# dfm/tinygp

Measured on AMD Instinct MI355X. Metric: GP log_probability evals/sec + Cholesky TFLOP/s (fp64), N=16,384, higher is better.
Workload: dtype f64; 1 GPU; c2: 1.5^2 ExpSquared(2.5), 1-D X, N=16384, fp64, diag=0.01, constant-density synthetic inputs (SURVEY 8d), dense Cholesky + tri-solve; n=16384, d=1, parallelism=single, nb_outer=1024

## Files before the change

tinygp_amd/csrc/capi.hip:

```cpp
#include <cmath>
#include <cstdlib>
#include <chrono>
#include <cstring>
#include <string>

#include "tgp_common.h"
#define CHAIN_HD __host__ __device__
#include "chain_tasks.h"
#define TILE_HD
#include "tile_order.h"

namespace tgp {

static thread_local std::string g_error;

void set_error(const char* fmt, ...) {
  char buf[1024];
  va_list ap;
  va_start(ap, fmt);
  vsnprintf(buf, sizeof(buf), fmt, ap);
  va_end(ap);
  g_error = buf;
}

// ... 239 lines not shown
  TGP_HIP_TRY(hipStreamSynchronize(ctx->stream));
  return TGP_OK;
}

static int64_t* option_slot(tgp_ctx* ctx, const char* key) {
  if (!strcmp(key, "nb_outer")) return &ctx->nb_outer;
  if (!strcmp(key, "lookahead")) return &ctx->lookahead;
  if (!strcmp(key, "profile")) return &ctx->profile;
  if (!strcmp(key, "first_split")) return &ctx->first_split;
  if (!strcmp(key, "first_small_tiles")) return &ctx->first_small_tiles;
  if (!strcmp(key, "keep_grad_buffers")) return &ctx->keep_grad_buffers;
  if (!strcmp(key, "stream_trsv")) return &ctx->stream_trsv;
  if (!strcmp(key, "trsv_groups")) return &ctx->trsv_groups;
  if (!strcmp(key, "nb_wide_rows")) return &ctx->nb_wide_rows;
  if (!strcmp(key, "dist_solve_aux")) return &ctx->dist_solve_aux;
  if (!strcmp(key, "solve_on_update")) return &ctx->solve_on_update;
  if (!strcmp(key, "fused_step")) return &ctx->fused_step;
  if (!strcmp(key, "chain_kernel")) return &ctx->chain_kernel;
  if (!strcmp(key, "chain_stamps")) return &ctx->chain_stamps;
  if (!strcmp(key, "chain_full_rows")) return &ctx->chain_full_rows;
  if (!strcmp(key, "chain_lds_pad")) return &ctx->chain_lds_pad;
  if (!strcmp(key, "chain_depth2")) return &ctx->chain_depth2;
  if (!strcmp(key, "chain_merged")) return &ctx->chain_merged;
  if (!strcmp(key, "chain_sub_panel")) return &ctx->chain_sub_panel;
  if (!strcmp(key, "chain_sub_min_rows")) return &ctx->chain_sub_min_rows;
  if (!strcmp(key, "chain_sub_role")) return &ctx->chain_sub_role;
  if (!strcmp(key, "chain_pre_wait")) return &ctx->chain_pre_wait;
  if (!strcmp(key, "chain_gate_split")) return &ctx->chain_gate_split;
  if (!strcmp(key, "chain_polls")) return &ctx->chain_polls;
  if (!strcmp(key, "chain_fwd_tasks")) return &ctx->chain_fwd_tasks;
  if (!strcmp(key, "chain_fast_update")) return &ctx->chain_fast_update;
  if (!strcmp(key, "chain_batch")) return &ctx->chain_batch;
  if (!strcmp(key, "chain_batch_lag")) return &ctx->chain_batch_lag;
  if (!strcmp(key, "chain_batch_rowlag")) return &ctx->chain_batch_rowlag;
  if (!strcmp(key, "chain_batch_minrows")) return &ctx->chain_batch_minrows;
  if (!strcmp(key, "kmat_plain_div")) return &ctx->kmat_plain_div;
  if (!strcmp(key, "chain_reserve")) return &ctx->chain_reserve;
  if (!strcmp(key, "gate_split")) return &ctx->gate_split;
  if (!strcmp(key, "reserve_max_tiles")) return &ctx->reserve_max_tiles;
  if (!strcmp(key, "sub_panel")) return &ctx->sub_panel;
  if (!strcmp(key, "sub_panel_min_rows")) return &ctx->sub_panel_min_rows;
  if (!strcmp(key, "nb_first")) return &ctx->nb_first;
  if (!strcmp(key, "split_tail")) return &ctx->split_tail;
  if (!strcmp(key, "gemm_role")) return &ctx->gemm_role;
  if (!strcmp(key, "host_join")) return &ctx->host_join;
  if (!strcmp(key, "late_join")) return &ctx->late_join;
// ... 998 lines not shown
```

tinygp_amd/csrc/chol.hip:

```cpp
#include <algorithm>
#include <atomic>
#include <functional>
#include <type_traits>

#include <thread>

#include "tgp_common.h"
#define CHAIN_HD __host__ __device__
#include "chain_tasks.h"

namespace tgp {

namespace {

typedef double d4 __attribute__((ext_vector_type(4)));
typedef float f4 __attribute__((ext_vector_type(4)));

template <typename T> struct Mfma;
template <> struct Mfma<double> {
  using acc_t = d4;
  static __device__ __forceinline__ acc_t mma(double a, double b, acc_t c) {
    return __builtin_amdgcn_mfma_f64_16x16x4f64(a, b, c, 0, 0, 0);
  }
  static __device__ __forceinline__ int drow(int lane, int r) { return (lane >> 4) + 4 * r; }
// ... 298 lines not shown
template <typename T> struct AgentBits;
template <> struct AgentBits<double> { using t = unsigned long long; };
template <> struct AgentBits<float> { using t = unsigned int; };
template <typename T>
__device__ __forceinline__ void st_agent(T* p, T v) {
  typename AgentBits<T>::t b;
  __builtin_memcpy(&b, &v, sizeof(T));
  __hip_atomic_store(reinterpret_cast<typename AgentBits<T>::t*>(p), b, __ATOMIC_RELAXED, __HIP_MEMORY_SCOPE_AGENT);
}

__device__ __forceinline__ void chain_stamp(long long* st, int k) {
  if (st != nullptr && threadIdx.x == 0) st[4 + k] = (long long)__builtin_amdgcn_s_memrealtime();
}

constexpr int CHAIN_FLAG_LD = 64;
constexpr uint32_t CHAIN_FINAL = 127;
constexpr int CHAIN_COLCNT_OFF = 16;
constexpr int CHAIN_QCNT_OFF = 96;
constexpr int CHAIN_XSTEP_OFF = 160;
constexpr int CHAIN_ZFLAG_OFF = 224;
constexpr int CHAIN_YSTATE_OFF = 288;
constexpr int CHAIN_TICKET_WORDS = CHAIN_YSTATE_OFF + int(CHAIN_MAX_ROW_TILES) / CHAIN_FWD_GROUP;
constexpr int CHAIN_PREFIX_OFF = CHAIN_TICKET_WORDS + 16;

template <typename T>
struct ChainArgs {
  T* A0;
  int64_t ld;
  T* dinv;
  int32_t* info;
  uint32_t* flags;
  int32_t* ticket;
  uint32_t epoch32;
  int32_t pivot_base;
  int32_t R;
  int32_t nblk;
  int32_t cb, ce;
  long long* stamps;
  int32_t launch;
  int32_t fast_update;
  const uint64_t* tasks;
  T* y;
  int32_t fgs;
  int32_t fprev;
  double* red;
  double* scal;
  int32_t red_total;
};

template <int NAP>
__device__ __forceinline__ void chain_wait(const uint32_t* f0, uint32_t v0, const uint32_t* f1, uint32_t v1,
                                           const uint32_t* f2, uint32_t v2, int32_t* info) {
  if (threadIdx.x < 64) {
    const int lane = threadIdx.x;
    const uint32_t* f = lane == 0 ? f0 : (lane == 1 ? f1 : (lane == 2 ? f2 : nullptr));
    const uint32_t want = lane == 0 ? v0 : (lane == 1 ? v1 : v2);
    bool ok = f == nullptr || __hip_atomic_load(f, __ATOMIC_RELAXED, __HIP_MEMORY_SCOPE_AGENT) == want;
    unsigned spin = 0;
    PollClock clk;
    while (!__all(ok)) {
      __builtin_amdgcn_s_sleep(NAP);
      if (!ok) ok = __hip_atomic_load(f, __ATOMIC_RELAXED, __HIP_MEMORY_SCOPE_AGENT) == want;
      bool dead = false;
      if ((spin & 255) == 255 && lane == 0)
        dead = clk.expired(spin) || poisoned(info);
      ++spin;
      if (__any(dead)) {
        if (lane == 0) atomicExch(info, STEP_TIMEOUT);
        break;
      }
    }
    if (lane == 0) __builtin_amdgcn_fence(__ATOMIC_ACQUIRE, "agent");
  }
  __syncthreads();
}

__device__ __forceinline__ void chain_publish(uint32_t* word, uint32_t value, int32_t* colcnt = nullptr) {
  asm volatile("s_waitcnt vmcnt(0)" ::: "memory");
  __syncthreads();
  if (threadIdx.x == 0) {
    __hip_atomic_store(word, value, __ATOMIC_RELAXED, __HIP_MEMORY_SCOPE_AGENT);
    if (colcnt != nullptr) __hip_atomic_fetch_add(colcnt, 1, __ATOMIC_RELAXED, __HIP_MEMORY_SCOPE_AGENT);
  }
}

// ... 782 lines not shown
    const ChainTask task = chain_unpack(q.tasks[t]);
    const int kind = task.kind, ti = task.i, tc = task.c, tk = task.k;
    s_task[5] = task.part;
    s_task[6] = task.k0;
    s_task[0] = kind; s_task[1] = ti; s_task[2] = tc; s_task[3] = tk;
  }
  __syncthreads();
  const int kind = __builtin_amdgcn_readfirstlane(s_task[0]);
  const int ti = __builtin_amdgcn_readfirstlane(s_task[1]);
  const int tc = __builtin_amdgcn_readfirstlane(s_task[2]);
  const int tk = __builtin_amdgcn_readfirstlane(s_task[3]);
  if (kind > 8) return;
  long long* st = nullptr;
  if (q.stamps != nullptr) {
    st = q.stamps + int64_t(__builtin_amdgcn_readfirstlane(s_task[4])) * 16;
    if (threadIdx.x == 0) {
      st[0] = kind; st[1] = kind == 1 ? tc : ti; st[2] = tc; st[3] = q.launch | (tk << 8) | (s_task[6] << 16);
      for (int k = 1; k < 12; ++k) st[4 + k] = 0;
    }
    chain_stamp(st, 0);
  }
  const uint32_t E = q.epoch32;
  const bool head_final = q.cb == 0;
  if (kind == 7) {
    const int c = tc;
    const int g = c / q.fgs;
    const bool prev = c > 0 || q.fprev != 0;
    chain_wait_counts(c - 1 > q.cb ? q.ticket + CHAIN_YSTATE_OFF + g : nullptr, c - 1 - q.cb,
                      (c == 0 && head_final) ? nullptr : reinterpret_cast<const int32_t*>(q.flags + c * CHAIN_FLAG_LD + c),
                      int32_t(E + CHAIN_FINAL), c > q.cb ? q.ticket + CHAIN_ZFLAG_OFF + (c - 1) : nullptr, 1, q.info);
    chain_stamp(st, 1);
    chain_fsolve<T>(q, S, c, prev);
    chain_stamp(st, 2);
    asm volatile("s_waitcnt vmcnt(0)" ::: "memory");
    __syncthreads();
    if (threadIdx.x == 0) __hip_atomic_store(q.ticket + CHAIN_ZFLAG_OFF + c, 1, __ATOMIC_RELAXED, __HIP_MEMORY_SCOPE_AGENT);
    chain_stamp(st, 3);
    return;
  }
  if (kind == 8) {
    const int c = tc, g = ti;
    const int target = q.R - c - ((c == 0 && head_final) ? 1 : 0);
    chain_wait_counts(q.ticket + CHAIN_COLCNT_OFF + c, target, q.ticket + CHAIN_ZFLAG_OFF + c, 1,
                      c > q.cb ? q.ticket + CHAIN_YSTATE_OFF + g : nullptr, c - q.cb, q.info);
    chain_stamp(st, 1);
    chain_fupdate<T>(q, S, c, g);
    chain_stamp(st, 2);
    asm volatile("s_waitcnt vmcnt(0)" ::: "memory");
    __syncthreads();
    if (threadIdx.x == 0)
      __hip_atomic_store(q.ticket + CHAIN_YSTATE_OFF + g, c - q.cb + 1, __ATOMIC_RELAXED, __HIP_MEMORY_SCOPE_AGENT);
    chain_stamp(st, 3);
    return;
  }
  if constexpr (sizeof(T) == 8) {
    if (kind == 6) {
      const int i = ti, c = tc, k = tk, k0 = __builtin_amdgcn_readfirstlane(s_task[6]);
      uint32_t* wt = q.flags + i * CHAIN_FLAG_LD + c;
      chain_wait<8>(q.flags + i * CHAIN_FLAG_LD + k, E + CHAIN_FINAL, q.flags + c * CHAIN_FLAG_LD + k, E + CHAIN_FINAL,
                    k0 > q.cb ? wt : nullptr, E + uint32_t(k0), q.info);
      chain_stamp(st, 1);
      chain_update_fast(q, S, i, c, k0, k + 1);
      chain_stamp(st, 2);
      chain_publish(wt, E + uint32_t(k + 1));
      chain_stamp(st, 3);
      return;
    }
  }
  if (kind >= 2 && kind <= 4) {
    const int i = ti, c = tc, k = tk;
    uint32_t* wt = q.flags + i * CHAIN_FLAG_LD + c;
    chain_wait<8>(q.flags + i * CHAIN_FLAG_LD + k, E + CHAIN_FINAL, q.flags + c * CHAIN_FLAG_LD + k, E + CHAIN_FINAL,
                  k > q.cb ? wt : nullptr, E + uint32_t(k), q.info);
    chain_stamp(st, 1);
    if (kind == 2) {
      if constexpr (sizeof(T) == 8) {
        if (q.fast_update) chain_update_fast(q, S, i, c, k, k + 1);
        else chain_update_full<T, 1>(q, S, i, c, k, 0);
      } else {
        chain_update_full<T, 1>(q, S, i, c, k, 0);
      }
    }
    else if (kind == 4) chain_update_full<T, CHAIN_CRIT_PARTS>(q, S, i, c, k, __builtin_amdgcn_readfirstlane(s_task[5]));
    else chain_update_diag<T>(q, S, c, k);
    chain_stamp(st, 2);
    if (kind == 4) {
      asm volatile("s_waitcnt vmcnt(0)" ::: "memory");
      __syncthreads();
      if (threadIdx.x == 0 &&
          __hip_atomic_fetch_add(q.ticket + CHAIN_QCNT_OFF + k, 1, __ATOMIC_RELAXED, __HIP_MEMORY_SCOPE_AGENT) ==
              CHAIN_CRIT_PARTS - 1)
        __hip_atomic_store(wt, E + uint32_t(k + 1), __ATOMIC_RELAXED, __HIP_MEMORY_SCOPE_AGENT);
    } else {
      chain_publish(wt, E + uint32_t(k + 1));
    }
    chain_stamp(st, 3);
    return;
  }
  __builtin_amdgcn_s_setprio(2);
  if (kind == 0) {
    const int i = ti, c = tc;
    uint32_t* wt = q.flags + i * CHAIN_FLAG_LD + c;
    const uint32_t* wl = q.flags + c * CHAIN_FLAG_LD + c;
    if (c > q.cb) chain_wait<4>(wt, E + uint32_t(c), nullptr, 0, nullptr, 0, q.info);
    acc_t V[8];
    chain_load_tile<T>(q, i, c, V);
    if (!(c == 0 && head_final)) chain_wait<4>(wl, E + CHAIN_FINAL, nullptr, 0, nullptr, 0, q.info);
    chain_stamp(st, 1);
    chain_solve<T>(q, S, i, c, V, st, 2);
    chain_publish(wt, E + CHAIN_FINAL, q.ticket + CHAIN_COLCNT_OFF + c);
    chain_stamp(st, 4);
    return;
  }
  const int c = tc;
  T* A = q.A0 + int64_t(c) * TILE * q.ld + int64_t(c) * TILE;
  const int64_t ld = q.ld;
  T* dinv = q.dinv + int64_t(c) * 2048;
  int32_t* info = q.info;
  const int32_t pivot_base = q.pivot_base + c * TILE;
  uint32_t* frow = q.flags + c * CHAIN_FLAG_LD;
  if (kind == 5) {
    acc_t Vx[8];
    if (c - 1 > q.cb) chain_wait<4>(frow + (c - 1), E + uint32_t(c - 1), nullptr, 0, nullptr, 0, q.info);
    chain_load_tile<T>(q, c, c - 1, Vx);
    chain_stamp(st, 1);
    const uint32_t* steps = c - 1 >= 1 ? q.flags + (c - 2) * CHAIN_FLAG_LD + (c - 1) : nullptr;
    int32_t* xstep = q.ticket + CHAIN_XSTEP_OFF + c;
    chain_xsolve_stream<T>(q, S, c, c - 1, Vx, steps, q.flags + (c - 1) * CHAIN_FLAG_LD + (c - 1), E, xstep);
    chain_stamp(st, 3);
    chain_publish(frow + (c - 1), E + CHAIN_FINAL, q.ticket + CHAIN_COLCNT_OFF + (c - 1));
    if (threadIdx.x == 0) __hip_atomic_store(xstep, 8, __ATOMIC_RELAXED, __HIP_MEMORY_SCOPE_AGENT);
    chain_stamp(st, 4);
    return;
  }
  acc_t Vx[8];
  acc_t Cfx[5];
  chain_fold_stream<T>(q, S, c, c - 1, Cfx, c > q.cb ? q.ticket + CHAIN_XSTEP_OFF + c : nullptr);
  chain_stamp(st, 3);
  if (c - 1 > q.cb) chain_wait<1>(frow + c, E + uint32_t(c - 1), nullptr, 0, nullptr, 0, q.info);
  else __syncthreads();
  chain_stamp(st, 5);
  {
    constexpr bool FOLD = true;
    uint32_t* step_word = q.flags + (c - 1) * CHAIN_FLAG_LD + c;
#define POTF2_ST(p, v) st_agent((p), T(v))
#define POTF2_V_IN_REGS Vx
#define POTF2_CF_IN_REGS Cfx
#define POTF2_PRE_SYNC(kb) do { if ((kb) >= 1) asm volatile("s_waitcnt vmcnt(0)" ::: "memory"); } while (0)
#define POTF2_POST_SYNC(kb)                                                                            \
  do {                                                                                                \
    if ((kb) >= 1 && threadIdx.x == 0)                                                                \
      __hip_atomic_store(step_word, E + uint32_t(kb), __ATOMIC_RELAXED, __HIP_MEMORY_SCOPE_AGENT);    \
  } while (0)
#include "potf2_body.inc"
#undef POTF2_POST_SYNC
#undef POTF2_PRE_SYNC
#undef POTF2_CF_IN_REGS
#undef POTF2_V_IN_REGS
#undef POTF2_ST
  }
  chain_stamp(st, 6);
  chain_publish(frow + c, E + CHAIN_FINAL, q.ticket + CHAIN_COLCNT_OFF + c);
// ... 721 lines not shown
  TGP_HIP_TRY(hipGetLastError());
  return TGP_OK;
}

template <typename T>
ChainPolicy chain_policy(const tgp_ctx* ctx) {
  if (sizeof(T) != 8 || ctx->chain_batch <= 1) return ChainPolicy{1, 1, 2, 0};
  return ChainPolicy{(int)ctx->chain_batch, (int)ctx->chain_batch_lag, (int)ctx->chain_batch_rowlag, (int)ctx->chain_batch_minrows};
}

template <typename T>
int launch_chain(tgp_ctx* ctx, hipStream_t st, T* A0, int64_t ld, T* dinv0, int64_t pivot_base, int64_t R,
                 int64_t nblk, int64_t cb, int64_t ce, bool head_done, hipEvent_t counters_ready, T* y0, bool fprev) {
  TGP_ARG_CHECK(R >= 1 && R <= CHAIN_MAX_ROW_TILES && cb >= 0 && cb < ce && ce <= nblk && nblk <= CHAIN_FLAG_LD && nblk <= R,
                "chain: bad panel shape (R=%lld, columns [%lld, %lld))", (long long)R, (long long)cb, (long long)ce);
  if (cb == 0 && !head_done) {
    TGP_TRY(launch_potf2<T>(ctx, st, A0, ld, dinv0, ctx->d_info, (int32_t)pivot_base));
    if (!ctx->trace) TGP_TRY(run_deferred_asm(ctx, st));
  }
  if (ctx->chain_polls_pending) {
    TGP_TRY(st_wait(ctx, st, ctx->ev_f));
    ctx->chain_polls_pending = false;
  }
  const int fwd = y0 != nullptr ? 1 : 0;
  int red = 0;
  if (fwd != 0 && ctx->chain_red_total > 0 && ctx->chain_red_total <= CHAIN_MAX_ROW_TILES && pivot_base % TILE == 0) {
    red = 1;
    ctx->chain_red_written += ce - cb;
    if (pivot_base / TILE + ce == ctx->chain_red_total && ctx->chain_red_written == ctx->chain_red_total) {
      red = 2;
      ctx->reductions_done = true;
    }
  }
  if (ctx->trace) {
    if (counters_ready != nullptr) TGP_TRY(ev_record(ctx, counters_ready, st));
    trace_push(ctx, 11, st, trace_off(ctx, A0), ld, R, cb, ce, nblk, fwd, red);
    return TGP_OK;
  }
  const ChainPolicy pol = chain_policy<T>(ctx);
  const std::array<int64_t, 9> key = {R, nblk, cb, ce, pol.batch, pol.lag, pol.rowlag, pol.minrows, fwd};
  auto found = ctx->chain_tables.find(key);
  if (found == ctx->chain_tables.end()) {
    const std::vector<ChainTask> list = chain_build((int)R, (int)nblk, (int)cb, (int)ce, pol, fwd, CHAIN_FWD_GROUP);
    tgp_ctx::ChainTable tab;
    tab.count = (int64_t)list.size();
    if (tab.count > 0) {
// ... 7 lines not shown
  const int64_t tasks = found->second.count;
  if (tasks == 0) {
    if (counters_ready != nullptr) TGP_TRY(ev_record(ctx, counters_ready, st));
    return TGP_OK;
  }
  ctx->step_epoch = (ctx->step_epoch + 1) & 0x1FFFFFFu;
  if (ctx->step_epoch == 0) ctx->step_epoch = 1;
  const uint32_t epoch = ctx->step_epoch;
  ChainArgs<T> q;
  q.A0 = A0; q.ld = ld; q.dinv = dinv0; q.info = ctx->d_info; q.flags = ctx->d_chain_flags;
  q.ticket = ctx->d_chain_ticket; q.epoch32 = epoch * 128u; q.pivot_base = (int32_t)pivot_base; q.R = (int32_t)R;
  q.nblk = (int32_t)nblk;
  q.cb = (int32_t)cb; q.ce = (int32_t)ce;
  q.stamps = nullptr;
  q.launch = (int32_t)ctx->chain_launches++;
  q.fast_update = (int32_t)ctx->chain_fast_update;
  q.tasks = found->second.dev;
  q.y = y0;
  q.fgs = CHAIN_FWD_GROUP;
  q.fprev = fprev ? 1 : 0;
  q.red = red != 0 ? ctx->d_chain_red : nullptr;
  q.scal = red != 0 ? ctx->d_scal : nullptr;
  q.red_total = red == 2 ? (int32_t)ctx->chain_red_total : 0;
  if (ctx->chain_stamps != 0 && ctx->chain_stamp_base + tasks <= CHAIN_STAMP_TASKS) {
    if (ctx->d_chain_stamps == nullptr)
      TGP_HIP_TRY(hipMalloc((void**)&ctx->d_chain_stamps, size_t(CHAIN_STAMP_TASKS) * 16 * sizeof(long long)));
    q.stamps = ctx->d_chain_stamps + ctx->chain_stamp_base * 16;
    ctx->chain_stamp_base += tasks;
  }
  TGP_HIP_TRY(hipMemsetAsync(ctx->d_chain_ticket, 0, size_t(CHAIN_TICKET_WORDS) * sizeof(int32_t), st));
  if (counters_ready != nullptr) TGP_TRY(ev_record(ctx, counters_ready, st));
  const size_t dyn = ctx->chain_lds_pad > 0 ? size_t(ctx->chain_lds_pad) + (sizeof(T) == 4 ? 36 * 256 * 4 : 0) : 0;
  hipLaunchKernelGGL((chain_kernel<T>), dim3((unsigned)tasks), dim3(512), dyn, st, q);
  TGP_HIP_TRY(hipGetLastError());
  return TGP_OK;
}

int launch_chain_poll(tgp_ctx* ctx, hipStream_t st, const void* A0, int64_t ld, int64_t R, int64_t c, bool first_external) {
  if (ctx->trace) {
    trace_push(ctx, 12, st, trace_off(ctx, static_cast<const double*>(A0)), ld, c);
    return TGP_OK;
  }
  const int32_t target = (int32_t)(R - c - ((c == 0 && first_external) ? 1 : 0));
  int32_t* count = ctx->d_chain_ticket + CHAIN_COLCNT_OFF + c;
  if (ctx->chain_polls == 3 && ctx->can_wait_value) {
    ctx->wait_values_inflight = true;
// ... 170 lines not shown
      if (S2 != S3 || !upd) TGP_TRY(st_wait(ctx, S2, ctx->ev_d));
      TGP_TRY(launch_trsv_fwd_step<T>(ctx, S2, mb, Ljj, ld, dj, y + j0));
    }
    if (need_mid) TGP_TRY(mid(ctx->ev_d));
    if (SB > 0 && j0 + TILE == sub_end && sub_end < k0 + kb) {
      const int64_t s0 = sub_end - SB, mr = n - sub_end, ncr = k0 + kb - sub_end;
      const T* P = A + s0 * ld + sub_end;
      const int64_t tiles = (mr / TILE) * (ncr / TILE) - (ncr / TILE) * (ncr / TILE - 1) / 2;
      TGP_TRY(launch_gemm_nt<T>(ctx, st, mr, ncr, SB, P, ld, P, ld, A + sub_end * ld + sub_end, ld, 1, 0,
                                tiles <= ctx->first_small_tiles ? 4 : 1));
    }
  }
  return TGP_OK;
}

template <typename T>
int potrf(tgp_ctx* ctx, int64_t n, T* A, int64_t ld, T* dinv, int32_t* info_host, T* y) {
  TGP_ARG_CHECK(n % TILE == 0 && ld >= n, "potrf: n must be a multiple of %d and ld >= n", TILE);
  if (info_host) *info_host = 0;
  if (n == 0) return TGP_OK;
  ctx->potf2_wait_counter = nullptr;
  ctx->prefix_hint_cols = 0;
  ctx->prefix_hint_counter = nullptr;
  ctx->reserve_hint = 0;
  hipStream_t S0 = ctx->stream, S1 = ctx->panel_stream;
  if (ctx->solve_on_update == 0 && y != nullptr) TGP_TRY(ensure_solve_stream(ctx));
  hipStream_t S2 = ctx->solve_on_update != 0 ? ctx->update_stream : ctx->solve_stream;
  if (y != nullptr) {
    TGP_TRY(ev_record(ctx, ctx->ev_c, S0));
    TGP_TRY(st_wait(ctx, S2, ctx->ev_c));
  }
  int64_t NB = ctx->nb_outer;
  if (NB < TILE) NB = TILE;
  NB = NB / TILE * TILE;
  if (!ctx->trace) TGP_HIP_TRY(hipMemsetAsync(ctx->d_info, 0, sizeof(int32_t), S0));
  ctx->chain_stamp_base = 0;
  ctx->chain_launches = 0;
  ctx->chain_polls_pending = false;
  const bool prof_on = ctx->profile != 0 && !ctx->trace;
  std::vector<ProfSpan> spans;
  ctx->ev_used = 0;
  hipEvent_t prof_t0 = nullptr;
  const bool span_dump = prof_on && getenv("TGP_SPAN_DUMP") != nullptr;
  if (prof_on) {
    TGP_TRY(prof_event(ctx, &prof_t0));
    TGP_HIP_TRY(hipEventRecord(prof_t0, S0));
// ... 65 lines not shown
    for (int64_t k0 = 0; k0 < n; k0 += width(k0)) s0.push_back(k0);
    s0.push_back(n);
    const int64_t P = (int64_t)s0.size() - 1;
    hipEvent_t ev_chain[2] = {ctx->ev_b, ctx->ev_g1}, ev_pfx[2] = {ctx->ev_g2, ctx->ev_e}, ev_T[2] = {ctx->ev_i, ctx->ev_j};
    const bool asm_side = ctx->asm_pending;
    ctx->asm_pending = false;
    if (P == 1 && !asm_side) {
      TGP_TRY(panel(S0, 0, s0[1] - s0[0], false, 0, no_mid));
      TGP_TRY(run_deferred_asm(ctx, nullptr));
    } else {
    TGP_TRY(ev_record(ctx, ctx->ev_a, S0));
    TGP_TRY(st_wait(ctx, S1, ctx->ev_a));
    TGP_TRY(panel(S1, 0, s0[1] - s0[0], false, 0, no_mid));
    TGP_TRY(run_deferred_asm(ctx, nullptr));
    TGP_TRY(ev_record(ctx, ev_chain[0], S1));
    for (int64_t p = 0; p + 1 < P; ++p) {
      const int64_t kb = s0[p + 1] - s0[p], next = s0[p + 1], wn = s0[p + 2] - s0[p + 1], mt = n - next;
      const T* Pp = A + s0[p] * ld + next;
      T* C = A + next * ld + next;
      TGP_TRY(st_wait(ctx, S0, ev_chain[p & 1]));
      if (p == 0 && asm_side) TGP_TRY(st_wait(ctx, S0, ctx->ev_asm));
      const bool prefix = wn < mt && ctx->chain_polls != 0;
      int32_t* counter = ctx->d_chain_ticket + CHAIN_PREFIX_OFF + (p & 3);
      if (prefix) {
        if (!ctx->trace) TGP_HIP_TRY(hipMemsetAsync(counter, 0, sizeof(int32_t), S0));
        TGP_TRY(ev_record(ctx, ev_pfx[p & 1], S0));
        ctx->prefix_hint_cols = wn;
        ctx->prefix_hint_counter = counter;
      }
      const int64_t t = mt / TILE;
      if (t * (t + 1) / 2 <= ctx->reserve_max_tiles) ctx->reserve_hint = ctx->chain_reserve;
      TGP_TRY(trailing(S0, mt, mt, kb, Pp, C, 0));
      if (!prefix) TGP_TRY(ev_record(ctx, ev_T[p & 1], S0));
      if (prefix) {
        const int64_t tm = mt / TILE, tp = wn / TILE;
        TGP_TRY(st_wait(ctx, S1, ev_pfx[p & 1]));
        if (ctx->trace || ctx->chain_polls == 2) {
          TGP_TRY(launch_prefix_poll(ctx, S1, counter, tp * tm - tp * (tp - 1) / 2, trace_off(ctx, C), ld));
        } else {
          ctx->potf2_wait_counter = counter;
          ctx->potf2_wait_target = tp * tm - tp * (tp - 1) / 2;
        }
      } else {
        TGP_TRY(st_wait(ctx, S1, ev_T[p & 1]));
      }
      if (p == 0 && asm_side) TGP_TRY(st_wait(ctx, S1, ctx->ev_asm));
      TGP_TRY(potf2_at(S1, next, false));
      TGP_TRY(chain_of_panel(S1, next, wn));
      TGP_TRY(ev_record(ctx, ev_chain[(p + 1) & 1], S1));
    }
    TGP_TRY(st_wait(ctx, S0, ev_chain[(P - 1) & 1]));
    }
  } else
  if (la && ctx->chain_kernel != 0 && ctx->chain_depth2 != 0) {
    std::vector<int64_t> s0;
    for (int64_t k0 = 0; k0 < n; k0 += width(k0)) s0.push_back(k0);
    s0.push_back(n);
    const int64_t P = (int64_t)s0.size() - 1;
    hipEvent_t ev_chain[2] = {ctx->ev_b, ctx->ev_g1}, ev_pre[2] = {ctx->ev_g2, ctx->ev_e};
    auto first_role = [&](int64_t m, int64_t nn) -> int {
      const int64_t tiles = (m / TILE) * (nn / TILE) - (nn / TILE) * (nn / TILE - 1) / 2;
      return tiles <= ctx->first_small_tiles ? 4 : 0;
    };
    const bool asm_side = ctx->asm_pending;
    ctx->asm_pending = false;
// ... 453 lines not shown
```

tinygp_amd/csrc/gemm.hip:

```cpp
#include <type_traits>

#include "tgp_common.h"

#define TILE_HD __host__ __device__
#include "tile_order.h"

namespace tgp {

namespace {

typedef double d4 __attribute__((ext_vector_type(4)));
typedef float f4 __attribute__((ext_vector_type(4)));

template <typename T> struct Mfma;
template <> struct Mfma<double> {
  using acc_t = d4;
  using v2_t = double __attribute__((ext_vector_type(2)));
  static __device__ __forceinline__ acc_t mma(double a, double b, acc_t c) {
    return __builtin_amdgcn_mfma_f64_16x16x4f64(a, b, c, 0, 0, 0);
  }
  static __device__ __forceinline__ int drow(int lane, int r) { return (lane >> 4) + 4 * r; }
};
template <> struct Mfma<float> {
  using acc_t = f4;
// ... 7 lines not shown
constexpr int BM = 128, BN = 128, BK = 16, LDS_LD = 144;

template <typename T>
struct GemmArgs {
  const T* A;
  const T* B;
  T* C;
  int64_t lda, ldb, ldc;
  int tm, tn;
  int k;
  int lower;
  int mode;
  int nblk;
  int skip00;
  int dG, dr, dl0, dnbt;
  int split_first, split_s, ngrid;
  T* ws;
  int* cnt;
  int batch;
  int64_t sA, sB, sC;
  int band;
  int prefix_tn = 0, prefix_cnt = 0;
  int32_t* prefix_done = nullptr;
};

__device__ __forceinline__ void decode_tile(int b, int tm, int tn, int lower, int& ti, int& tj, int band = 0) {
  tile_decode(b, tm, tn, lower, band, ti, tj);
}

template <typename T>
__device__ __forceinline__ void decode_tile_dist(int b, const GemmArgs<T>& g, int& ti, int& tj, int& gt) {
  int q = 0, g0 = (g.dl0 * g.dG + g.dr) * g.dnbt;
  const int step = g.dG * g.dnbt, tri = g.dnbt * (g.dnbt - 1) / 2;
  for (;;) {
    const int cnt = g.dnbt * (g.tm - g0) - tri;
    if (b < cnt) break;
    b -= cnt;
    g0 += step;
    ++q;
  }
  int tir, s;
  decode_tile(b, g.tm - g0, g.dnbt, 1, tir, s, g.band);
  ti = g0 + tir;
  tj = q * g.dnbt + s;
  gt = g0 + s;
}

template <typename T, int ROLE>
__global__ __launch_bounds__(256, 2) void gemm_nt_kernel(GemmArgs<T> g) {
  constexpr int SBUF = sizeof(T) == 8 ? 2 * BK * LDS_LD : 3 * BK * BM;
  __shared__ __attribute__((aligned(16))) T sAm[SBUF];
  __shared__ __attribute__((aligned(16))) T sBm[SBUF];
  T(*sA)[BK * LDS_LD] = reinterpret_cast<T(*)[BK * LDS_LD]>(sAm);
  T(*sB)[BK * LDS_LD] = reinterpret_cast<T(*)[BK * LDS_LD]>(sBm);

  if (ROLE == 1) __builtin_amdgcn_s_setprio(1);
  for (int tile = blockIdx.x; tile < (ROLE == 2 ? g.ngrid : g.nblk); tile += gridDim.x) {
  int bid = tile;
  int slice = 0, nsl = 1, tail_idx = 0;
  if (ROLE == 2 && tile >= g.split_first) {
    tail_idx = (tile - g.split_first) / g.split_s;
    slice = (tile - g.split_first) % g.split_s;
    nsl = g.split_s;
    bid = g.split_first + tail_idx;
  }
  const bool in_prefix = g.prefix_cnt > 0 && bid < g.prefix_cnt;
  {
    const int base = g.prefix_cnt > 0 ? (in_prefix ? 0 : g.prefix_cnt) : 0;
    const int cnt = g.prefix_cnt > 0 ? (in_prefix ? g.prefix_cnt : g.nblk - g.prefix_cnt) : g.nblk;
    const int loc = bid - base;
    const int nx = 8, q = cnt / nx, r = cnt % nx;
    const int xcd = loc % nx, idx = loc / nx;
    bid = base + (xcd < r ? xcd * (q + 1) : r * (q + 1) + (xcd - r) * q) + idx;
  }
  int ti, tj, gt;
  const T* gA = g.A;
  const T* gB = g.B;
  T* gC = g.C;
  if constexpr (ROLE == 3) {
    const int xcd = tile & 7, idx = tile >> 3, slot = idx & 63;
    const int pk = (idx >> 6) * 8 + xcd;
    const int ptm = (g.tm + 7) >> 3, ptn = (g.tn + 7) >> 3;
    const int pps = g.lower ? (ptm * (ptm + 1)) / 2 : ptm * ptn;
    const int pl = pk / g.batch, q = pk - pl * g.batch;
    if (pl >= pps) return;
    int Pi, Pj;
    if (g.lower) {
      Pi = int((sqrtf(8.0f * float(pl) + 1.0f) - 1.0f) * 0.5f);
      while (Pi > 0 && (Pi * (Pi + 1)) / 2 > pl) --Pi;
      while (((Pi + 1) * (Pi + 2)) / 2 <= pl) ++Pi;
// ... 181 lines not shown
#pragma unroll
          for (int b = 0; b < 4; ++b) {
            char* cb = const_cast<char*>(Cu) + (int64_t(a * 16) * g.ldc + b * 16) * 8;
#pragma unroll
            for (int t = 0; t < 4; ++t) *reinterpret_cast<double*>(cb + voff[t]) = cc[b][t];
          }
        }
      }
    } else
    if (pipe) {
      if (ROLE == 0 && in_prefix) {
#pragma unroll
        for (int a = 0; a < 4; ++a) {
#pragma unroll
          for (int b = 0; b < 4; ++b) {
            const char* cb = Cu + (int64_t(a * 16) * g.ldc + b * 16) * 8;
#pragma unroll
            for (int t = 0; t < 4; ++t)
              asm volatile("global_store_dwordx2 %0, %1, %2 sc1" ::"v"(voff[t]), "v"(acc[a][b][t]), "s"(cb) : "memory");
          }
        }
        asm volatile("s_waitcnt vmcnt(0)" ::: "memory");
        __syncthreads();
        if (tid == 0) __hip_atomic_fetch_add(g.prefix_done, 1, __ATOMIC_RELAXED, __HIP_MEMORY_SCOPE_AGENT);
      } else {
#pragma unroll
      for (int a = 0; a < 4; ++a) {
#pragma unroll
        for (int b = 0; b < 4; ++b) {
          char* cb = const_cast<char*>(Cu) + (int64_t(a * 16) * g.ldc + b * 16) * 8;
#pragma unroll
          for (int t = 0; t < 4; ++t) *reinterpret_cast<double*>(cb + voff[t]) = acc[a][b][t];
        }
      }
      }
    } else if (g.mode == 0) {
#pragma unroll
      for (int ap = 0; ap < 4; ap += 2) {
        T* col[2];
        double c[2][4][4];
#pragma unroll
        for (int a = 0; a < 2; ++a) {
          col[a] = Cb + int64_t((ap + a) * 16 + 4 * lq + lk) * g.ldc;
#pragma unroll
          for (int b = 0; b < 4; ++b)
#pragma unroll
            for (int t = 0; t < 4; ++t) c[a][b][t] = col[a][b * 16 + rot[t]];
// ... 98 lines not shown
              acc[a][b] = __builtin_amdgcn_mfma_f32_32x32x2f32(aop[a], bop[b], acc[a][b], 0, 0, 0);
        }
        stage = stage == NST - 1 ? 0 : stage + 1;
      }
    };
    kloop();
    if (g.mode == 0) {
#pragma unroll
      for (int a = 0; a < 2; ++a)
#pragma unroll
        for (int b = 0; b < 2; ++b) acc[a][b] = -acc[a][b];
    }
    if (ROLE == 0 && in_prefix) {
#pragma unroll
      for (int a = 0; a < 2; ++a)
#pragma unroll
        for (int b = 0; b < 2; ++b)
#pragma unroll
          for (int r = 0; r < 16; ++r)
            __hip_atomic_store(reinterpret_cast<uint32_t*>(centry(a, b, r)), __float_as_uint(acc[a][b][r]), __ATOMIC_RELAXED,
                               __HIP_MEMORY_SCOPE_AGENT);
      asm volatile("s_waitcnt vmcnt(0)" ::: "memory");
      __syncthreads();
      if (tid == 0) __hip_atomic_fetch_add(g.prefix_done, 1, __ATOMIC_RELAXED, __HIP_MEMORY_SCOPE_AGENT);
    } else {
#pragma unroll
    for (int a = 0; a < 2; ++a)
#pragma unroll
      for (int b = 0; b < 2; ++b)
#pragma unroll
        for (int r = 0; r < 16; ++r) *centry(a, b, r) = acc[a][b][r];
    }
  }
  }
}

constexpr int SM = 64, S_LD = 80;

template <typename T>
__global__ __launch_bounds__(256) __attribute__((amdgpu_waves_per_eu(3))) void gemm_nt_small_kernel(GemmArgs<T> g) {
  using M = Mfma<T>;
  using acc_t = typename M::acc_t;
  using v2_t = typename M::v2_t;
  constexpr int SBUF = sizeof(T) == 8 ? 3 * BK * SM : 2 * BK * S_LD;
  __shared__ __attribute__((aligned(16))) T sAm[SBUF];
  __shared__ __attribute__((aligned(16))) T sBm[SBUF];
  T(*sA)[BK * S_LD] = reinterpret_cast<T(*)[BK * S_LD]>(sAm);
// ... 246 lines not shown

}

static unsigned persistent_grid(const tgp_ctx* ctx, int nblk, int64_t reserve) {
  if (reserve <= 0) return unsigned(nblk);
  int64_t slots = 2 * int64_t(ctx->cus > 0 ? ctx->cus : 256) - reserve;
  slots = slots / 8 * 8;
  if (slots < 8) slots = 8;
  return unsigned(nblk <= slots ? nblk : slots);
}

template <typename T>
int launch_gemm_nt(tgp_ctx* ctx, hipStream_t st, int64_t m, int64_t n, int64_t k, const T* A,
                   int64_t lda, const T* B, int64_t ldb, T* C, int64_t ldc, int lower, int mode,
                   int role) {
  TGP_ARG_CHECK(m % BM == 0 && n % BN == 0 && k % BK == 0 && k > 0,
                "gemm_nt: m,n must be multiples of %d and k of %d (got %lld,%lld,%lld)", BM, BK,
                (long long)m, (long long)n, (long long)k);
  if (m == 0 || n == 0) return TGP_OK;
  if (ctx->trace) {
    const int64_t pfx = role == 0 ? ctx->prefix_hint_cols / BN : 0;
    ctx->prefix_hint_cols = 0;
    ctx->prefix_hint_counter = nullptr;
    if (role == 0) ctx->reserve_hint = 0;
    trace_push(ctx, 3, st, trace_off(ctx, A), trace_off(ctx, B), trace_off(ctx, C), m, n, k,
               int64_t(lower) | (int64_t(role) << 8) | (pfx << 16), ldc);
    return TGP_OK;
  }
  GemmArgs<T> g;
  g.skip00 = 0;
  g.dG = g.dr = g.dl0 = g.dnbt = 0;
  g.split_first = 0; g.split_s = 1; g.ngrid = 0; g.ws = nullptr; g.cnt = nullptr;
  g.batch = 1; g.sA = g.sB = g.sC = 0;
  g.band = (int)ctx->tile_band;
  g.prefix_tn = g.prefix_cnt = 0;
  g.prefix_done = nullptr;
  TGP_ARG_CHECK(role != 3 || (k <= 256 && mode == 0), "role 3 needs the small-tile path");
  if ((((role == 1 || role == 3) && k <= 256) || role == 4 || role == 5) && (mode == 0 || mode == 1)) {
    g.skip00 = (role == 3 || role == 5);
    g.A = A; g.B = B; g.C = C;
    g.lda = lda; g.ldb = ldb; g.ldc = ldc;
    g.tm = int(m / SM); g.tn = int(n / SM);
    g.k = int(k); g.lower = lower; g.mode = mode;
    if (lower) {
      if (g.tn > g.tm) g.tn = g.tm;
      g.nblk = g.tn * g.tm - (g.tn * (g.tn - 1)) / 2;
    } else {
      g.nblk = g.tm * g.tn;
    }
    hipLaunchKernelGGL((gemm_nt_small_kernel<T>), dim3((unsigned)g.nblk), dim3(256), 0, st, g);
    TGP_HIP_TRY(hipGetLastError());
    return TGP_OK;
  }
  g.A = A; g.B = B; g.C = C;
  g.lda = lda; g.ldb = ldb; g.ldc = ldc;
  g.tm = int(m / BM); g.tn = int(n / BN);
  g.k = int(k); g.lower = lower; g.mode = mode;
  if (lower) {
    if (g.tn > g.tm) g.tn = g.tm;
    g.nblk = g.tn * g.tm - (g.tn * (g.tn - 1)) / 2;
  } else {
    g.nblk = g.tm * g.tn;
  }
  const int64_t reserve = role == 0 ? ctx->reserve_hint : 0;
  ctx->reserve_hint = 0;
  if (role == 0 && ctx->prefix_hint_cols > 0) {
    TGP_ARG_CHECK(lower && mode == 0 && m == n && ctx->prefix_hint_cols % BN == 0 && ctx->prefix_hint_cols < n &&
                      k / BK >= 8 && ctx->prefix_hint_counter != nullptr,
                  "gemm_nt: a prefix needs a lower square update with at least 128 k-columns");
    g.prefix_tn = int(ctx->prefix_hint_cols / BN);
    g.prefix_cnt = tile_count(g.tm, g.prefix_tn, 1);
    g.prefix_done = ctx->prefix_hint_counter;
  }
  ctx->prefix_hint_cols = 0;
  ctx->prefix_hint_counter = nullptr;
  g.split_first = g.nblk; g.split_s = 1; g.ngrid = g.nblk; g.ws = nullptr; g.cnt = nullptr;
  if (ctx->split_tail != 0 && role == 0 && mode == 0 && reserve <= 0 && sizeof(T) == 8 && st == ctx->stream && g.prefix_cnt == 0) {
    const int slots = 2 * (ctx->cus > 0 ? ctx->cus : 256);
    const int R = g.nblk % slots, nkt = g.k / BK;
    int S = 1;
    while (R > 0 && 2 * S * R <= slots && 2 * S <= 8 && nkt % (2 * S) == 0 && nkt / (2 * S) >= 8) S *= 2;
    if (S > 1) {
      const size_t need = size_t(slots) * BM * BN * sizeof(T) + size_t(slots) * sizeof(int);
      if (ctx->gemm_ws_bytes < need) {
        if (ctx->d_gemm_ws) TGP_HIP_TRY(hipFree(ctx->d_gemm_ws));
        ctx->d_gemm_ws = nullptr;
        ctx->gemm_ws_bytes = 0;
        TGP_HIP_TRY(hipMalloc(&ctx->d_gemm_ws, need));
        TGP_HIP_TRY(hipMemset(ctx->d_gemm_ws, 0, need));
        ctx->gemm_ws_bytes = need;
      }
      g.split_first = g.nblk - R;
      g.split_s = S;
      g.ngrid = g.split_first + R * S;
      g.ws = static_cast<T*>(ctx->d_gemm_ws);
      g.cnt = reinterpret_cast<int*>(static_cast<char*>(ctx->d_gemm_ws) + size_t(slots) * BM * BN * sizeof(T));
      hipLaunchKernelGGL((gemm_nt_kernel<T, 2>), dim3(unsigned(g.ngrid)), dim3(256), 0, st, g);
      TGP_HIP_TRY(hipGetLastError());
// ... 128 lines not shown
```

tinygp_amd/csrc/tgp_common.h:

```cpp
#pragma once

#include <hip/hip_runtime.h>

#include <cstdarg>
#include <cstdint>
#include <cstdio>
#include <chrono>
#include <array>
#include <functional>
#include <map>
#include <mutex>
#include <vector>

#include "../../include/tgp_hip.h"

namespace tgp {

constexpr int TILE = TGP_TILE;
constexpr int SUB = 16;

void set_error(const char* fmt, ...);

#define TGP_HIP_TRY(expr)                                                                  \
  do {                                                                                     \
// ... 69 lines not shown
  int64_t trsv_groups = 0;
  int64_t keep_grad_buffers = 0;
  int64_t first_small_tiles = 1100;
  int64_t fused_step = 0;
  int64_t chain_reserve = 96;
  int64_t reserve_max_tiles = 1200;
  int64_t gate_split = 1;
  int64_t sub_panel = 0;
  int64_t sub_panel_min_rows = 0;
  int64_t nb_first = 0;
  int64_t split_tail = 0;
  int64_t gemm_role = 1;
  int64_t late_join = 1;
  int64_t chain_reduce = 1;
  double* d_chain_red = nullptr;
  int64_t chain_red_total = 0;
  int64_t chain_red_written = 0;
  bool reductions_done = false;
  bool defer_join = false;
  bool join_deferred = false;
  int64_t reserve_hint = 0;
  int64_t prefix_hint_cols = 0;
  int32_t* prefix_hint_counter = nullptr;
  const int32_t* potf2_wait_counter = nullptr;
  int64_t potf2_wait_target = 0;
  uint32_t* d_step_flag = nullptr;
  uint32_t step_epoch = 0;
  int64_t chain_kernel = 1;
  uint32_t* d_chain_flags = nullptr;
  int32_t* d_chain_ticket = nullptr;
  int64_t chain_fast_update = 0;
  int64_t chain_batch = 1;
  int64_t chain_batch_lag = 1;
  int64_t chain_batch_rowlag = 4;
  int64_t chain_batch_minrows = 32;
  struct ChainTable {
    uint64_t* dev = nullptr;
    int64_t count = 0;
  };
  std::map<std::array<int64_t, 9>, ChainTable> chain_tables;
  int64_t chain_full_rows = 4096;
  int64_t chain_depth2 = 1;
  int64_t chain_merged = 1;
  int64_t chain_sub_panel = 0;
  int64_t chain_sub_min_rows = 0;
  int64_t chain_sub_role = 4;
  int64_t kmat_plain_div = 0;
  int64_t chain_polls = 1;
  int64_t chain_fwd_tasks = 1;
  bool chain_fwd_now = false;
  bool wait_values_inflight = false;
  int64_t tile_band = 8;
  int64_t asm_defer = 0;
  std::function<int()> deferred_asm;
  hipEvent_t ev_asm_gate = nullptr;
  int64_t fault_inject = 0;
  int64_t host_join = 1;
  bool serializing_tool = false;
  hipStream_t rescue_stream = nullptr;
  hipEvent_t ev_join = nullptr;
  bool has_device = false;
  bool can_wait_value = false;
  int64_t poll_timeout_ms = 4000;
  int64_t timeout_retries = 0;
  int64_t chain_pre_wait = 0;
  int64_t chain_gate_split = 0;
// ... 227 lines not shown
```

Baseline: 39.85 evals/s.

## Gate tail chain tasks per column on trailing-update completion counters

For the last trailing update before the chained tail factorisation, the GEMM now bumps a per-column completion counter instead of a single prefix counter. The chain kernel starts without waiting for the whole update event, and each task polls its column's counter until all tiles in that column are done. This lets the tail Cholesky overlap with the end of the trailing GEMM rather than serialising on it. In exchange it adds extra polling lanes and atomics, and it disables the banded tile order for that launch.

New measurement: 39.96 evals/s (median of 6 runs). No clear change (+0.3%).

```diff
diff --git a/tinygp_amd/csrc/capi.hip b/tinygp_amd/csrc/capi.hip
--- a/tinygp_amd/csrc/capi.hip
+++ b/tinygp_amd/csrc/capi.hip
@@ -285,6 +285,8 @@
   if (!strcmp(key, "chain_lds_pad")) return &ctx->chain_lds_pad;
   if (!strcmp(key, "chain_depth2")) return &ctx->chain_depth2;
   if (!strcmp(key, "chain_merged")) return &ctx->chain_merged;
+  if (!strcmp(key, "chain_tail_prefix")) return &ctx->chain_tail_prefix;
+  if (!strcmp(key, "tail_prefix_launches")) return &ctx->tail_prefix_launches;
   if (!strcmp(key, "chain_sub_panel")) return &ctx->chain_sub_panel;
   if (!strcmp(key, "chain_sub_min_rows")) return &ctx->chain_sub_min_rows;
   if (!strcmp(key, "chain_sub_role")) return &ctx->chain_sub_role;
diff --git a/tinygp_amd/csrc/chol.hip b/tinygp_amd/csrc/chol.hip
--- a/tinygp_amd/csrc/chol.hip
+++ b/tinygp_amd/csrc/chol.hip
@@ -344,6 +344,8 @@
 constexpr int CHAIN_YSTATE_OFF = 288;
 constexpr int CHAIN_TICKET_WORDS = CHAIN_YSTATE_OFF + int(CHAIN_MAX_ROW_TILES) / CHAIN_FWD_GROUP;
 constexpr int CHAIN_PREFIX_OFF = CHAIN_TICKET_WORDS + 16;
+constexpr int CHAIN_COLGATE_OFF = CHAIN_PREFIX_OFF + 16;
+static_assert((CHAIN_COLGATE_OFF + CHAIN_FLAG_LD) * sizeof(int32_t) <= 4096, "d_chain_ticket is 4 096 bytes (capi.hip)");
 
 template <typename T>
 struct ChainArgs {
@@ -368,21 +370,27 @@
   double* red;
   double* scal;
   int32_t red_total;
+  const int32_t* gate;
 };
 
 template <int NAP>
 __device__ __forceinline__ void chain_wait(const uint32_t* f0, uint32_t v0, const uint32_t* f1, uint32_t v1,
-                                           const uint32_t* f2, uint32_t v2, int32_t* info) {
+                                           const uint32_t* f2, uint32_t v2, int32_t* info, const int32_t* fg = nullptr,
+                                           int32_t vg = 0) {
   if (threadIdx.x < 64) {
     const int lane = threadIdx.x;
-    const uint32_t* f = lane == 0 ? f0 : (lane == 1 ? f1 : (lane == 2 ? f2 : nullptr));
-    const uint32_t want = lane == 0 ? v0 : (lane == 1 ? v1 : v2);
-    bool ok = f == nullptr || __hip_atomic_load(f, __ATOMIC_RELAXED, __HIP_MEMORY_SCOPE_AGENT) == want;
+    const uint32_t* f = lane == 0 ? f0 : (lane == 1 ? f1 : (lane == 2 ? f2 : (lane == 3 ? reinterpret_cast<const uint32_t*>(fg) : nullptr)));
+    const uint32_t want = lane == 0 ? v0 : (lane == 1 ? v1 : (lane == 2 ? v2 : uint32_t(vg)));
+    auto ready = [&]() {
+      const uint32_t v = __hip_atomic_load(f, __ATOMIC_RELAXED, __HIP_MEMORY_SCOPE_AGENT);
+      return lane == 3 ? int32_t(v) >= int32_t(want) : v == want;
+    };
+    bool ok = f == nullptr || ready();
     unsigned spin = 0;
     PollClock clk;
     while (!__all(ok)) {
       __builtin_amdgcn_s_sleep(NAP);
-      if (!ok) ok = __hip_atomic_load(f, __ATOMIC_RELAXED, __HIP_MEMORY_SCOPE_AGENT) == want;
+      if (!ok) ok = ready();
       bool dead = false;
       if ((spin & 255) == 255 && lane == 0)
         dead = clk.expired(spin) || poisoned(info);
@@ -1211,6 +1219,9 @@
   }
   const uint32_t E = q.epoch32;
   const bool head_final = q.cb == 0;
+  const int gcol = kind == 5 ? tc - 1 : tc;
+  const int32_t* gate = (q.gate != nullptr && kind <= 6) ? q.gate + gcol : nullptr;
+  const int32_t gate_want = q.R - gcol;
   if (kind == 7) {
     const int c = tc;
     const int g = c / q.fgs;
@@ -1247,7 +1258,7 @@
       const int i = ti, c = tc, k = tk, k0 = __builtin_amdgcn_readfirstlane(s_task[6]);
       uint32_t* wt = q.flags + i * CHAIN_FLAG_LD + c;
       chain_wait<8>(q.flags + i * CHAIN_FLAG_LD + k, E + CHAIN_FINAL, q.flags + c * CHAIN_FLAG_LD + k, E + CHAIN_FINAL,
-                    k0 > q.cb ? wt : nullptr, E + uint32_t(k0), q.info);
+                    k0 > q.cb ? wt : nullptr, E + uint32_t(k0), q.info, gate, gate_want);
       chain_stamp(st, 1);
       chain_update_fast(q, S, i, c, k0, k + 1);
       chain_stamp(st, 2);
@@ -1260,7 +1271,7 @@
     const int i = ti, c = tc, k = tk;
     uint32_t* wt = q.flags + i * CHAIN_FLAG_LD + c;
     chain_wait<8>(q.flags + i * CHAIN_FLAG_LD + k, E + CHAIN_FINAL, q.flags + c * CHAIN_FLAG_LD + k, E + CHAIN_FINAL,
-                  k > q.cb ? wt : nullptr, E + uint32_t(k), q.info);
+                  k > q.cb ? wt : nullptr, E + uint32_t(k), q.info, gate, gate_want);
     chain_stamp(st, 1);
     if (kind == 2) {
       if constexpr (sizeof(T) == 8) {
@@ -1291,7 +1302,8 @@
     const int i = ti, c = tc;
     uint32_t* wt = q.flags + i * CHAIN_FLAG_LD + c;
     const uint32_t* wl = q.flags + c * CHAIN_FLAG_LD + c;
-    if (c > q.cb) chain_wait<4>(wt, E + uint32_t(c), nullptr, 0, nullptr, 0, q.info);
+    if (c > q.cb || gate != nullptr)
+      chain_wait<4>(c > q.cb ? wt : nullptr, E + uint32_t(c), nullptr, 0, nullptr, 0, q.info, gate, gate_want);
     acc_t V[8];
     chain_load_tile<T>(q, i, c, V);
     if (!(c == 0 && head_final)) chain_wait<4>(wl, E + CHAIN_FINAL, nullptr, 0, nullptr, 0, q.info);
@@ -1310,7 +1322,8 @@
   uint32_t* frow = q.flags + c * CHAIN_FLAG_LD;
   if (kind == 5) {
     acc_t Vx[8];
-    if (c - 1 > q.cb) chain_wait<4>(frow + (c - 1), E + uint32_t(c - 1), nullptr, 0, nullptr, 0, q.info);
+    if (c - 1 > q.cb || gate != nullptr)
+      chain_wait<4>(c - 1 > q.cb ? frow + (c - 1) : nullptr, E + uint32_t(c - 1), nullptr, 0, nullptr, 0, q.info, gate, gate_want);
     chain_load_tile<T>(q, c, c - 1, Vx);
     chain_stamp(st, 1);
     const uint32_t* steps = c - 1 >= 1 ? q.flags + (c - 2) * CHAIN_FLAG_LD + (c - 1) : nullptr;
@@ -1326,7 +1339,8 @@
   acc_t Cfx[5];
   chain_fold_stream<T>(q, S, c, c - 1, Cfx, c > q.cb ? q.ticket + CHAIN_XSTEP_OFF + c : nullptr);
   chain_stamp(st, 3);
-  if (c - 1 > q.cb) chain_wait<1>(frow + c, E + uint32_t(c - 1), nullptr, 0, nullptr, 0, q.info);
+  if (c - 1 > q.cb || gate != nullptr)
+    chain_wait<1>(c - 1 > q.cb ? frow + c : nullptr, E + uint32_t(c - 1), nullptr, 0, nullptr, 0, q.info, gate, gate_want);
   else __syncthreads();
   chain_stamp(st, 5);
   {
@@ -2094,6 +2108,9 @@
     TGP_TRY(st_wait(ctx, st, ctx->ev_f));
     ctx->chain_polls_pending = false;
   }
+  const int32_t* gate = ctx->chain_gate_hint;
+  ctx->chain_gate_hint = nullptr;
+  TGP_ARG_CHECK(gate == nullptr || (cb == 0 && ce == nblk && nblk == R), "chain: only a launch over the whole rest is gated per column");
   const int fwd = y0 != nullptr ? 1 : 0;
   int red = 0;
   if (fwd != 0 && ctx->chain_red_total > 0 && ctx->chain_red_total <= CHAIN_MAX_ROW_TILES && pivot_base % TILE == 0) {
@@ -2147,6 +2164,7 @@
   q.red = red != 0 ? ctx->d_chain_red : nullptr;
   q.scal = red != 0 ? ctx->d_scal : nullptr;
   q.red_total = red == 2 ? (int32_t)ctx->chain_red_total : 0;
+  q.gate = gate;
   if (ctx->chain_stamps != 0 && ctx->chain_stamp_base + tasks <= CHAIN_STAMP_TASKS) {
     if (ctx->d_chain_stamps == nullptr)
       TGP_HIP_TRY(hipMalloc((void**)&ctx->d_chain_stamps, size_t(CHAIN_STAMP_TASKS) * 16 * sizeof(long long)));
@@ -2363,6 +2381,8 @@
   ctx->potf2_wait_counter = nullptr;
   ctx->prefix_hint_cols = 0;
   ctx->prefix_hint_counter = nullptr;
+  ctx->prefix_hint_stride = 0;
+  ctx->chain_gate_hint = nullptr;
   ctx->reserve_hint = 0;
   hipStream_t S0 = ctx->stream, S1 = ctx->panel_stream;
   if (ctx->solve_on_update == 0 && y != nullptr) TGP_TRY(ensure_solve_stream(ctx));
@@ -2474,16 +2494,27 @@
       if (p == 0 && asm_side) TGP_TRY(st_wait(ctx, S0, ctx->ev_asm));
       const bool prefix = wn < mt && ctx->chain_polls != 0;
       int32_t* counter = ctx->d_chain_ticket + CHAIN_PREFIX_OFF + (p & 3);
+      const int64_t t = mt / TILE;
+      const bool reserved = t * (t + 1) / 2 <= ctx->reserve_max_tiles && ctx->chain_reserve > 0;
+      const bool tail = wn == mt && ctx->chain_polls != 0 && ctx->chain_tail_prefix != 0 && !ctx->trace && reserved &&
+                        t <= CHAIN_FLAG_LD;
+      int32_t* colcnt = ctx->d_chain_ticket + CHAIN_COLGATE_OFF;
+      if (tail) {
+        TGP_HIP_TRY(hipMemsetAsync(colcnt, 0, size_t(t) * sizeof(int32_t), S0));
+        TGP_TRY(ev_record(ctx, ev_pfx[p & 1], S0));
+        ctx->prefix_hint_cols = wn;
+        ctx->prefix_hint_counter = colcnt;
+        ctx->prefix_hint_stride = 1;
+      }
       if (prefix) {
         if (!ctx->trace) TGP_HIP_TRY(hipMemsetAsync(counter, 0, sizeof(int32_t), S0));
         TGP_TRY(ev_record(ctx, ev_pfx[p & 1], S0));
         ctx->prefix_hint_cols = wn;
         ctx->prefix_hint_counter = counter;
       }
-      const int64_t t = mt / TILE;
       if (t * (t + 1) / 2 <= ctx->reserve_max_tiles) ctx->reserve_hint = ctx->chain_reserve;
       TGP_TRY(trailing(S0, mt, mt, kb, Pp, C, 0));
-      if (!prefix) TGP_TRY(ev_record(ctx, ev_T[p & 1], S0));
+      if (!prefix && !tail) TGP_TRY(ev_record(ctx, ev_T[p & 1], S0));
       if (prefix) {
         const int64_t tm = mt / TILE, tp = wn / TILE;
         TGP_TRY(st_wait(ctx, S1, ev_pfx[p & 1]));
@@ -2493,6 +2524,16 @@
           ctx->potf2_wait_counter = counter;
           ctx->potf2_wait_target = tp * tm - tp * (tp - 1) / 2;
         }
+      } else if (tail) {
+        TGP_TRY(st_wait(ctx, S1, ev_pfx[p & 1]));
+        if (ctx->chain_polls == 2) {
+          TGP_TRY(launch_prefix_poll(ctx, S1, colcnt, t, trace_off(ctx, C), ld));
+        } else {
+          ctx->potf2_wait_counter = colcnt;
+          ctx->potf2_wait_target = t;
+        }
+        ctx->chain_gate_hint = colcnt;
+        ctx->tail_prefix_launches++;
       } else {
         TGP_TRY(st_wait(ctx, S1, ev_T[p & 1]));
       }
diff --git a/tinygp_amd/csrc/gemm.hip b/tinygp_amd/csrc/gemm.hip
--- a/tinygp_amd/csrc/gemm.hip
+++ b/tinygp_amd/csrc/gemm.hip
@@ -53,6 +53,7 @@
   int band;
   int prefix_tn = 0, prefix_cnt = 0;
   int32_t* prefix_done = nullptr;
+  int prefix_stride = 0;
 };
 
 __device__ __forceinline__ void decode_tile(int b, int tm, int tn, int lower, int& ti, int& tj, int band = 0) {
@@ -96,7 +97,7 @@
     bid = g.split_first + tail_idx;
   }
   const bool in_prefix = g.prefix_cnt > 0 && bid < g.prefix_cnt;
-  {
+  if (g.prefix_stride == 0) {
     const int base = g.prefix_cnt > 0 ? (in_prefix ? 0 : g.prefix_cnt) : 0;
     const int cnt = g.prefix_cnt > 0 ? (in_prefix ? g.prefix_cnt : g.nblk - g.prefix_cnt) : g.nblk;
     const int loc = bid - base;
@@ -324,7 +325,7 @@
         }
         asm volatile("s_waitcnt vmcnt(0)" ::: "memory");
         __syncthreads();
-        if (tid == 0) __hip_atomic_fetch_add(g.prefix_done, 1, __ATOMIC_RELAXED, __HIP_MEMORY_SCOPE_AGENT);
+        if (tid == 0) __hip_atomic_fetch_add(g.prefix_done + tj * g.prefix_stride, 1, __ATOMIC_RELAXED, __HIP_MEMORY_SCOPE_AGENT);
       } else {
 #pragma unroll
       for (int a = 0; a < 4; ++a) {
@@ -469,7 +470,7 @@
                                __HIP_MEMORY_SCOPE_AGENT);
       asm volatile("s_waitcnt vmcnt(0)" ::: "memory");
       __syncthreads();
-      if (tid == 0) __hip_atomic_fetch_add(g.prefix_done, 1, __ATOMIC_RELAXED, __HIP_MEMORY_SCOPE_AGENT);
+      if (tid == 0) __hip_atomic_fetch_add(g.prefix_done + tj * g.prefix_stride, 1, __ATOMIC_RELAXED, __HIP_MEMORY_SCOPE_AGENT);
     } else {
 #pragma unroll
     for (int a = 0; a < 2; ++a)
@@ -762,6 +763,7 @@
     const int64_t pfx = role == 0 ? ctx->prefix_hint_cols / BN : 0;
     ctx->prefix_hint_cols = 0;
     ctx->prefix_hint_counter = nullptr;
+    ctx->prefix_hint_stride = 0;
     if (role == 0) ctx->reserve_hint = 0;
     trace_push(ctx, 3, st, trace_off(ctx, A), trace_off(ctx, B), trace_off(ctx, C), m, n, k,
                int64_t(lower) | (int64_t(role) << 8) | (pfx << 16), ldc);
@@ -805,15 +807,23 @@
   const int64_t reserve = role == 0 ? ctx->reserve_hint : 0;
   ctx->reserve_hint = 0;
   if (role == 0 && ctx->prefix_hint_cols > 0) {
-    TGP_ARG_CHECK(lower && mode == 0 && m == n && ctx->prefix_hint_cols % BN == 0 && ctx->prefix_hint_cols < n &&
-                      k / BK >= 8 && ctx->prefix_hint_counter != nullptr,
+    const bool per_col = ctx->prefix_hint_stride != 0;
+    TGP_ARG_CHECK(lower && mode == 0 && m == n && ctx->prefix_hint_cols % BN == 0 &&
+                      (per_col ? ctx->prefix_hint_cols == n : ctx->prefix_hint_cols < n) && k / BK >= 8 &&
+                      ctx->prefix_hint_counter != nullptr,
                   "gemm_nt: a prefix needs a lower square update with at least 128 k-columns");
+    TGP_ARG_CHECK(!per_col || (reserve > 0 && g.tn <= 64), "gemm_nt: a per-column prefix needs the persistent grid and <= 64 tile columns");
     g.prefix_tn = int(ctx->prefix_hint_cols / BN);
     g.prefix_cnt = tile_count(g.tm, g.prefix_tn, 1);
     g.prefix_done = ctx->prefix_hint_counter;
+    if (per_col) {
+      g.prefix_stride = 1;
+      g.band = 0;
+    }
   }
   ctx->prefix_hint_cols = 0;
   ctx->prefix_hint_counter = nullptr;
+  ctx->prefix_hint_stride = 0;
   g.split_first = g.nblk; g.split_s = 1; g.ngrid = g.nblk; g.ws = nullptr; g.cnt = nullptr;
   if (ctx->split_tail != 0 && role == 0 && mode == 0 && reserve <= 0 && sizeof(T) == 8 && st == ctx->stream && g.prefix_cnt == 0) {
     const int slots = 2 * (ctx->cus > 0 ? ctx->cus : 256);
diff --git a/tinygp_amd/csrc/tgp_common.h b/tinygp_amd/csrc/tgp_common.h
--- a/tinygp_amd/csrc/tgp_common.h
+++ b/tinygp_amd/csrc/tgp_common.h
@@ -115,6 +115,8 @@
   int64_t reserve_hint = 0;
   int64_t prefix_hint_cols = 0;
   int32_t* prefix_hint_counter = nullptr;
+  int64_t prefix_hint_stride = 0;
+  const int32_t* chain_gate_hint = nullptr;
   const int32_t* potf2_wait_counter = nullptr;
   int64_t potf2_wait_target = 0;
   uint32_t* d_step_flag = nullptr;
@@ -135,6 +137,8 @@
   int64_t chain_full_rows = 4096;
   int64_t chain_depth2 = 1;
   int64_t chain_merged = 1;
+  int64_t chain_tail_prefix = 1;
+  int64_t tail_prefix_launches = 0;
   int64_t chain_sub_panel = 0;
   int64_t chain_sub_min_rows = 0;
   int64_t chain_sub_role = 4;
```
